# romanoshiliarhopoulos/Backgammon-Engine

Measured on AMD Instinct MI355X. Metric: self-play env steps/sec @65k concurrent games, higher is better.
Workload: dtype f32; 1 GPU; config3: 65 536 concurrent games per MI355X, greedy 198->128->1 value net (tdgammonNEW100k weights), auto-reset, Philox dice; games_per_gpu=65536, burnin_steps=160, parallelism=shard1, games_finished=2250605

## Files before the change

backgammon-engine_amd/csrc/bg_eval.h:

```cpp
#pragma once
#include "bg_board.h"
#include "bg_td_plan.h"

namespace bg {

constexpr int N_IN = 198, N_HID = 128;
constexpr int N_PARAMS = N_HID * N_IN + N_HID + N_HID + 1;
constexpr int K_STEPS = N_IN / 2;
constexpr int EVAL_LDS_BYTES = K_STEPS * 64 * 16;
constexpr int EVAL_THREADS = 768;

typedef float floatx16 __attribute__((ext_vector_type(16)));

__device__ __forceinline__ float fast_sigmoid(float x)
{
    return __builtin_amdgcn_rcpf(1.0f + __builtin_amdgcn_exp2f(-1.44269504088896340736f * x));
}

__device__ __forceinline__ void best_atomic_max(unsigned long long *__restrict__ best, uint32_t game, float v, uint32_t key_turn,
                                                bool valid, int width)
{
    const int lane = threadIdx.x & 63;
    uint32_t bits = __float_as_uint(v);
    bits = (key_turn >> 31) ? ~bits : bits;
// ... 415 lines not shown
            const uint32_t sd = mover ^ (uint32_t)pass;
            const uint32_t b0 = sd ? p[4] : p[0], b1 = sd ? p[5] : p[1], b2 = sd ? p[6] : p[2], b3 = sd ? p[7] : p[3];
            const uint32_t c0 = sd ? q[4] : q[0], c1 = sd ? q[5] : q[1], c2 = sd ? q[6] : q[2], c3 = sd ? q[7] : q[3];
            const uint32_t diff = (b0 ^ c0) | (b1 ^ c1) | (b2 ^ c2) | (b3 ^ c3);
            if (pass == 1 && __ballot(diff != 0u) == 0ull) break;
            const uint32_t ge_new[3] = {b0 | b1 | b2 | b3, b1 | b2 | b3, (b0 & b1) | b2 | b3};
            const uint32_t ge_old[3] = {c0 | c1 | c2 | c3, c1 | c2 | c3, (c0 & c1) | c2 | c3};
            const uint32_t side4 = 4u * sd;
#pragma unroll
            for (int k = 0; k < 3; ++k) {
                uint32_t x = (ge_new[k] ^ ge_old[k]) & PTS;
                while (x) {
                    const int pos = __ffs(x) - 1; x &= x - 1;
                    BG_PUSH(delta_row_board(pos - 1, 0) + side4 + (uint32_t)k, 0, ((ge_new[k] >> pos) & 1u) ? 1 : -1);
                }
            }
            uint32_t x4 = diff & PTS & ((b2 | b3) | (c2 | c3));
            const Side sn{{b0, b1, b2, b3}}, so{{c0, c1, c2, c3}};
            while (x4) {
                const int pos = __ffs(x4) - 1; x4 &= x4 - 1;
                const int n1 = count_at(sn, pos), n0 = count_at(so, pos);
                const int d = (n1 > 3 ? n1 - 3 : 0) - (n0 > 3 ? n0 - 3 : 0);
                if (d) BG_PUSH(delta_row_board(pos - 1, 0) + side4 + 3u, 1, d);
            }
            if (diff & 1u) {
                const int d = count_at(sn, 0) - count_at(so, 0);
                BG_PUSH(sd ? (uint32_t)delta_row(197) : (uint32_t)delta_row(194), 1, sd ? 2 * d : d);
            }
            if (diff & (1u << 25)) {
                const int d = count_at(sn, 25) - count_at(so, 25);
                BG_PUSH(sd ? (uint32_t)delta_row(195) : (uint32_t)delta_row(196), 1, sd ? d : 2 * d);
            }
        }
#else
#pragma unroll
        for (int sd = 0; sd < 2; ++sd) {
            const uint32_t b0 = p[4 * sd], b1 = p[4 * sd + 1], b2 = p[4 * sd + 2], b3 = p[4 * sd + 3];
            const uint32_t c0 = q[4 * sd], c1 = q[4 * sd + 1], c2 = q[4 * sd + 2], c3 = q[4 * sd + 3];
            const uint32_t diff = (b0 ^ c0) | (b1 ^ c1) | (b2 ^ c2) | (b3 ^ c3);
            const uint32_t ge_new[3] = {b0 | b1 | b2 | b3, b1 | b2 | b3, (b0 & b1) | b2 | b3};
            const uint32_t ge_old[3] = {c0 | c1 | c2 | c3, c1 | c2 | c3, (c0 & c1) | c2 | c3};
#pragma unroll
            for (int k = 0; k < 3; ++k) {
                uint32_t x = (ge_new[k] ^ ge_old[k]) & PTS;
                while (x) {
                    const int pos = __ffs(x) - 1; x &= x - 1;
                    BG_PUSH(delta_row_board(pos - 1, 4 * sd + k), 0, ((ge_new[k] >> pos) & 1u) ? 1 : -1);
                }
            }
            uint32_t x4 = diff & PTS & ((b2 | b3) | (c2 | c3));
            const Side sn{{b0, b1, b2, b3}}, so{{c0, c1, c2, c3}};
            while (x4) {
                const int pos = __ffs(x4) - 1; x4 &= x4 - 1;
                const int n1 = count_at(sn, pos), n0 = count_at(so, pos);
                const int d = (n1 > 3 ? n1 - 3 : 0) - (n0 > 3 ? n0 - 3 : 0);
                if (d) BG_PUSH(delta_row_board(pos - 1, 4 * sd + 3), 1, d);
            }
            if (diff & 1u) {
                const int d = count_at(sn, 0) - count_at(so, 0);
                BG_PUSH(delta_row(sd == 0 ? 194 : 197), sd == 0 ? 1 : 2, d);
            }
            if (diff & (1u << 25)) {
                const int d = count_at(sn, 25) - count_at(so, 25);
                BG_PUSH(delta_row(sd == 0 ? 196 : 195), sd == 0 ? 2 : 1, d);
            }
        }
#endif
        }
#undef BG_PUSH
        if (cnt > DELTA_MAX) { cnt = DELTA_MAX; list_overflow = true; }
        n_delta += cnt;
        uint32_t maxcnt = 0;
#pragma unroll
        for (int b = 4; b >= 0; --b) {
            const uint32_t t = maxcnt | (1u << b);
            if (__ballot(cnt >= t) != 0ull) maxcnt = t;
        }
#if defined(BG_ABL) && (BG_ABL & 2)
        maxcnt = maxcnt > 100 ? 1 : 0;
#endif
        __builtin_amdgcn_wave_barrier();

        f32x2_t sum2 = {0.0f, 0.0f};
        const f32x4_t *w2v = reinterpret_cast<const f32x4_t *>(sW2);
        const uint32_t sW_lds = (uint32_t)(uintptr_t)(__attribute__((address_space(3))) float4 *)sW;
#pragma unroll 1
        for (int c = 0; c < 2; ++c) {
            f32x2_t a[16], a2[16];
#if defined(BG_ABL) && (BG_ABL & 8)
#pragma unroll
            for (int j = 0; j < 16; ++j) { a[j] = (f32x2_t){0.25f * (float)j, 0.5f}; a2[j] = (f32x2_t){0.125f, -0.25f * (float)j}; }
            (void)ah;
#else
#pragma unroll
            for (int j = 0; j < 8; ++j) { const f32x4_t t = ah[16 * c + j]; a[2 * j] = t.lo; a[2 * j + 1] = t.hi; }
#pragma unroll
            for (int j = 0; j < 8; ++j) { const f32x4_t t = ah[16 * c + 8 + j]; a2[2 * j] = t.lo; a2[2 * j + 1] = t.hi; }
#endif
            if (c == 1) { nr0 = root_rows[2 * (long long)nxi.x]; nr1 = root_rows[2 * (long long)nxi.x + 1]; }
            uint32_t ent = lst[0];
            for (uint32_t e = 0; e < maxcnt; ++e) {
                const uint32_t nent = lst[(e + 1 < DELTA_MAX ? e + 1 : e) * 64];
                f32x2_t d2;
                uint32_t addr;
                delta_entry(ent, sW_lds + 256u * (uint32_t)c, d2, addr);
                delta_apply_32<0>(a, d2, addr);
                delta_apply_32<128>(a2, d2, addr);
                ent = nent;
            }
#if defined(BG_ABL) && (BG_ABL & 4)
#define BG_SIGP(A, W, S) __builtin_elementwise_fma(W, A, S)
#else
#define BG_SIGP(A, W, S) delta_sigmoid_pair(A, W, S)
#endif
#pragma unroll
            for (int j = 0; j < 8; ++j) {
                const f32x4_t w = w2v[16 * c + j];
                sum2 = BG_SIGP(a[2 * j], w.lo, sum2);
                sum2 = BG_SIGP(a[2 * j + 1], w.hi, sum2);
            }
#pragma unroll
            for (int j = 0; j < 8; ++j) {
                const f32x4_t w = w2v[16 * c + 8 + j];
                sum2 = BG_SIGP(a2[2 * j], w.lo, sum2);
                sum2 = BG_SIGP(a2[2 * j + 1], w.hi, sum2);
            }
#undef BG_SIGP
        }
        const float sum = sum2.x + sum2.y;
        __builtin_amdgcn_wave_barrier();
        {
            const float v = fast_sigmoid(sum + b2);
            if (valid) values[row] = v;
            best_atomic_max(best, __shfl(inf.x, inv, 64), __shfl(v, inv, 64), __shfl(inf.y, inv, 64), __shfl((int)valid, inv, 64) != 0, 64);
        }
        tile = next_tile;
    }
    __shared__ unsigned int s_nd;
    if (threadIdx.x == 0) s_nd = 0;
    __syncthreads();
    {
        uint32_t t = n_delta;
#pragma unroll
        for (int m = 1; m < 64; m <<= 1) t += __shfl_xor(t, m, 64);
        if (lane == 0 && t) atomicAdd(&s_nd, t);
    }
    __syncthreads();
    if (delta_counter && threadIdx.x == 0 && s_nd) atomicAdd(delta_counter, (unsigned long long)s_nd);
    if (err_word && __ballot(list_overflow) != 0ull && lane == 0) atomicOr(err_word, err_bit);
#ifdef BG_EVAL_WGCLOCK
    if (n_rows_ptr && threadIdx.x == 0) {
        values[n_rows_imm - 1 - (long long)blockIdx.x] = (float)(wall_clock64() - wg_t0) * 0.01f;
        values[n_rows_imm - 1 - (long long)gridDim.x - (long long)blockIdx.x] = (float)s_ticket;
    }
#endif
}

constexpr int K16_STEPS = 13;
constexpr int EVAL16_W_BYTES = K16_STEPS * 4 * 64 * 16;
constexpr int EVAL16_LUT_BYTES = 16 * 8;
constexpr int EVAL16_LDS_TOTAL = EVAL16_W_BYTES + EVAL16_LUT_BYTES + (EVAL_THREADS / 64) * EVAL_RED_FLOATS * 4;
typedef __bf16 bf16x8 __attribute__((ext_vector_type(8)));

__host__ __device__ inline uint16_t f32_to_bf16_rne(float f)
{
    union { float f; uint32_t u; } c{f};
    return (uint16_t)((c.u + 0x7FFFu + ((c.u >> 16) & 1u)) >> 16);
}

inline void relayout_w1_bf16(const float *w1, uint16_t *wl)
{
    for (int s = 0; s < K16_STEPS; ++s)
        for (int c = 0; c < 4; ++c)
            for (int l = 0; l < 64; ++l)
                for (int j = 0; j < 8; ++j) {
                    const int f = 16 * s + 8 * (l >> 5) + j;
                    wl[((s * 4 + c) * 64 + l) * 8 + j] = f < N_IN ? f32_to_bf16_rne(w1[(32 * c + (l & 31)) * N_IN + f]) : 0;
                }
}
inline void make_count_lut(uint32_t *lut )
{
    for (int n = 0; n < 16; ++n) {
        const uint16_t e0 = n >= 1 ? 0x3F80 : 0, e1 = n >= 2 ? 0x3F80 : 0, e2 = n >= 3 ? 0x3F80 : 0;
        const uint16_t e3 = n >= 4 ? f32_to_bf16_rne(0.5f * (float)(n - 3)) : 0;
        lut[2 * n] = (uint32_t)e0 | ((uint32_t)e1 << 16);
        lut[2 * n + 1] = (uint32_t)e2 | ((uint32_t)e3 << 16);
    }
}

__global__ __launch_bounds__(EVAL_THREADS) void eval_rows_bf16_kernel(
    const uint4 *__restrict__ rows, const unsigned long long *__restrict__ n_rows_ptr, long long n_rows_imm,
    unsigned long long *__restrict__ rows_eval_counter, const uint4 *__restrict__ wl16, const uint2 *__restrict__ lut,
    const float *__restrict__ b1, const float *__restrict__ w2, const float *__restrict__ b2p, float *__restrict__ values,
    const uint2 *__restrict__ info, unsigned long long *__restrict__ best)
{
    extern __shared__ uint4 sW16[];
    uint2 *sLut = reinterpret_cast<uint2 *>(sW16 + K16_STEPS * 4 * 64);
    float *sRed = reinterpret_cast<float *>(sLut + 16) + (threadIdx.x >> 6) * EVAL_RED_FLOATS;
    for (int i = threadIdx.x; i < K16_STEPS * 4 * 64; i += EVAL_THREADS) sW16[i] = wl16[i];
    if (threadIdx.x < 16) sLut[threadIdx.x] = lut[threadIdx.x];
    __syncthreads();

    long long n_rows = n_rows_imm;
    if (n_rows_ptr) { const long long c = (long long)*n_rows_ptr; n_rows = c < n_rows_imm ? c : n_rows_imm; }
    if (rows_eval_counter && blockIdx.x == 0 && threadIdx.x == 0) atomicAdd(rows_eval_counter, (unsigned long long)n_rows);
    const long long n_tiles = (n_rows + 31) >> 5;
    const int lane = threadIdx.x & 63;
    const int r = lane & 31, h = lane >> 5;
    const long long wave = (long long)blockIdx.x * (EVAL_THREADS / 64) + (threadIdx.x >> 6);
    const long long n_waves = (long long)gridDim.x * (EVAL_THREADS / 64);
    constexpr float NL2E = -1.44269504088896340736f;
    float b1s[4], w2v[4];
#pragma unroll
    for (int c = 0; c < 4; ++c) { b1s[c] = NL2E * b1[32 * c + r]; w2v[c] = w2[32 * c + r]; }
    const float b2 = *b2p;

    uint4 nx0 = make_uint4(0, 0, 0, 0), nx1 = make_uint4(0, 0, 0, 0);
    if (wave < n_tiles && wave * 32 + r < n_rows) { nx0 = rows[2 * (wave * 32 + r)]; nx1 = rows[2 * (wave * 32 + r) + 1]; }

    for (long long tile = wave; tile < n_tiles; tile += n_waves) {
        const uint32_t p[8] = {nx0.x, nx0.y, nx0.z, nx0.w, nx1.x, nx1.y, nx1.z, nx1.w};
        {
            const long long nrow = (tile + n_waves) * 32 + r;
            nx0 = make_uint4(0, 0, 0, 0); nx1 = make_uint4(0, 0, 0, 0);
            if (nrow < n_rows) { nx0 = rows[2 * nrow]; nx1 = rows[2 * nrow + 1]; }
        }
        const Side sa{{p[0], p[1], p[2], p[3]}}, sb{{p[4], p[5], p[6], p[7]}};
        floatx16 acc0 = {0}, acc1 = {0}, acc2 = {0}, acc3 = {0};
        const uint4 *wp = sW16 + lane;
#pragma unroll 4
        for (int s = 0; s < 12; ++s) {
            const int pos = 2 * s + h + 1;
            const uint2 l0 = sLut[count_at(sa, pos)], l1 = sLut[count_at(sb, pos)];
            union { uint4 u; bf16x8 v; } a, w0, w1, w2r, w3;
            a.u = make_uint4(l0.x, l0.y, l1.x, l1.y);
            w0.u = wp[(s * 4 + 0) * 64]; w1.u = wp[(s * 4 + 1) * 64]; w2r.u = wp[(s * 4 + 2) * 64]; w3.u = wp[(s * 4 + 3) * 64];
            acc0 = __builtin_amdgcn_mfma_f32_32x32x16_bf16(a.v, w0.v, acc0, 0, 0, 0);
            acc1 = __builtin_amdgcn_mfma_f32_32x32x16_bf16(a.v, w1.v, acc1, 0, 0, 0);
            acc2 = __builtin_amdgcn_mfma_f32_32x32x16_bf16(a.v, w2r.v, acc2, 0, 0, 0);
            acc3 = __builtin_amdgcn_mfma_f32_32x32x16_bf16(a.v, w3.v, acc3, 0, 0, 0);
        }
        {
            const int turn = (p[0] & TURN_BIT) ? 1 : 0;
            const uint32_t t0 = turn == 0 ? 0x3F80u : 0u, t1 = turn == 0 ? 0u : 0x3F80u;
            const uint32_t bar1 = f32_to_bf16_rne(0.5f * (float)count_at(sa, 0)), bar2 = f32_to_bf16_rne(0.5f * (float)count_at(sb, 25));
            const uint32_t off1 = f32_to_bf16_rne((float)count_at(sa, 25) / 15.0f), off2 = f32_to_bf16_rne((float)count_at(sb, 0) / 15.0f);
            union { uint4 u; bf16x8 v; } a, w0, w1, w2r, w3;
            a.u = h ? make_uint4(0, 0, 0, 0) : make_uint4(t0 | (t1 << 16), bar1 | (bar2 << 16), off1 | (off2 << 16), 0u);
            w0.u = wp[(12 * 4 + 0) * 64]; w1.u = wp[(12 * 4 + 1) * 64]; w2r.u = wp[(12 * 4 + 2) * 64]; w3.u = wp[(12 * 4 + 3) * 64];
            acc0 = __builtin_amdgcn_mfma_f32_32x32x16_bf16(a.v, w0.v, acc0, 0, 0, 0);
            acc1 = __builtin_amdgcn_mfma_f32_32x32x16_bf16(a.v, w1.v, acc1, 0, 0, 0);
            acc2 = __builtin_amdgcn_mfma_f32_32x32x16_bf16(a.v, w2r.v, acc2, 0, 0, 0);
            acc3 = __builtin_amdgcn_mfma_f32_32x32x16_bf16(a.v, w3.v, acc3, 0, 0, 0);
        }
        float part[16];
#pragma unroll
        for (int j = 0; j < 16; ++j) {
            const float s0 = __builtin_amdgcn_rcpf(1.0f + __builtin_amdgcn_exp2f(__builtin_fmaf(acc0[j], NL2E, b1s[0])));
            const float s1 = __builtin_amdgcn_rcpf(1.0f + __builtin_amdgcn_exp2f(__builtin_fmaf(acc1[j], NL2E, b1s[1])));
            const float s2 = __builtin_amdgcn_rcpf(1.0f + __builtin_amdgcn_exp2f(__builtin_fmaf(acc2[j], NL2E, b1s[2])));
            const float s3 = __builtin_amdgcn_rcpf(1.0f + __builtin_amdgcn_exp2f(__builtin_fmaf(acc3[j], NL2E, b1s[3])));
            part[j] = w2v[0] * s0 + w2v[1] * s1 + w2v[2] * s2 + w2v[3] * s3;
        }
#pragma unroll
        for (int q = 0; q < 4; ++q)
#pragma unroll
            for (int j = 0; j < 4; ++j) sRed[r * EVAL_RED_STRIDE + 8 * q + 4 * h + j] = part[4 * q + j];
        __builtin_amdgcn_wave_barrier();
        float sum = 0.0f;
#pragma unroll
        for (int c = 0; c < 16; ++c) sum += sRed[(16 * h + c) * EVAL_RED_STRIDE + r];
        sum += __shfl_xor(sum, 32, 64);
        __builtin_amdgcn_wave_barrier();
        {
            const long long orow = tile * 32 + r;
            const bool vrow = h == 0 && orow < n_rows;
            const float v = fast_sigmoid(sum + b2);
            if (vrow) values[orow] = v;
            if (info) {
                const uint2 inf = vrow ? info[orow] : make_uint2(0u, 0u);
                best_atomic_max(best, inf.x, v, inf.y, vrow, 32);
            }
        }
    }
}

#ifndef BG_ROOT3_PHASE_STEPS
#define BG_ROOT3_PHASE_STEPS 7
#endif
constexpr int ROOT3_PHASE_STEPS = BG_ROOT3_PHASE_STEPS;
constexpr int ROOT3_PHASES = (K16_STEPS + ROOT3_PHASE_STEPS - 1) / ROOT3_PHASE_STEPS;
constexpr int ROOT3_PART_U4 = K16_STEPS * 4 * 64;
constexpr int ROOT3_LDS_TOTAL = 3 * ROOT3_PHASE_STEPS * 4 * 64 * 16 + EVAL16_LUT_BYTES;

inline void relayout_w1_bf16x3(const float *w1, uint16_t *wl)
{
    static const int tail_map[8] = {192, 193, 194, 195, 196, 197, -1, -1};
    for (int s = 0; s < K16_STEPS; ++s)
        for (int c = 0; c < 4; ++c)
            for (int l = 0; l < 64; ++l)
                for (int j = 0; j < 8; ++j) {
                    int f = 16 * s + 8 * (l >> 5) + j;
                    if (s == 12) f = (l >> 5) == 0 ? tail_map[j] : -1;
                    float w = f >= 0 && f < N_IN ? w1[(32 * c + (l & 31)) * N_IN + f] : 0.0f;
                    if (f >= 196) w = w / 15.0f;
                    const size_t o = (((size_t)s * 4 + c) * 64 + l) * 8 + j;
// ... 386 lines not shown
```

backgammon-engine_amd/csrc/bg_root_resident.h:

```cpp
#pragma once
#include "bg_eval.h"

namespace bg {

constexpr int D16_XBUF_U4 = K16_STEPS * 64;

#ifndef BG_ROOT_F16X2
#define BG_ROOT_F16X2 1
#endif
#if BG_ROOT_F16X2
constexpr int ROOT_PLANES = 2;
typedef f16x8 root_vec8;
#define BG_ROOT_MFMA(A, B, C) __builtin_amdgcn_mfma_f32_32x32x16_f16(A, B, C, 0, 0, 0)
__device__ __forceinline__ uint32_t root_half_bits(float x) { return (uint32_t)f16_bits((_Float16)x); }
constexpr uint32_t ROOT_ONE = 0x3C00u;
#else
constexpr int ROOT_PLANES = 3;
typedef bf16x8 root_vec8;
#define BG_ROOT_MFMA(A, B, C) __builtin_amdgcn_mfma_f32_32x32x16_bf16(A, B, C, 0, 0, 0)
__device__ __forceinline__ uint32_t root_half_bits(float x) { return (uint32_t)f32_to_bf16_rne(x); }
constexpr uint32_t ROOT_ONE = 0x3F80u;
#endif
constexpr bool ROOT_F16X2 = BG_ROOT_F16X2 != 0;

__host__ __device__ inline bool w1_fits_f16_split(float w, _Float16 &hi, _Float16 &lo)
{
    const float aw = w < 0.0f ? -w : w;
    hi = (_Float16)w;
    lo = (_Float16)(w - (float)hi);
    const float res = w - ((float)hi + (float)lo);
    return aw < 65504.0f
           && (res < 0.0f ? -res : res) <= aw * 4.76837158e-7f + 5.96046448e-8f;
}

inline int relayout_w1_f16x2_root(const float *w1, uint16_t *wl)
{
    static const int tail_map[8] = {192, 193, 194, 195, 196, 197, -1, -1};
    int rc = 0;
    for (int s = 0; s < K16_STEPS; ++s)
        for (int c = 0; c < 4; ++c)
            for (int l = 0; l < 64; ++l)
                for (int j = 0; j < 8; ++j) {
                    int f = 16 * s + 8 * (l >> 5) + j;
                    if (s == 12) f = (l >> 5) == 0 ? tail_map[j] : -1;
                    float w = f >= 0 && f < N_IN ? w1[(32 * c + (l & 31)) * N_IN + f] : 0.0f;
                    if (f >= 196) w = w / 15.0f;
                    _Float16 hi, lo;
                    if (!w1_fits_f16_split(w, hi, lo)) rc = -1;
                    const size_t o = (((size_t)s * 4 + c) * 64 + l) * 8 + j;
                    wl[o] = f16_bits(hi);
                    wl[(size_t)ROOT3_PART_U4 * 8 + o] = f16_bits(lo);
                }
    return rc;
}

constexpr int ROOTR_THREADS = 256;
constexpr int ROOTR_LDS_BYTES = 2 * D16_XBUF_U4 * 16 + EVAL16_LUT_BYTES + 3 * 1024;

__global__ __launch_bounds__(ROOTR_THREADS, 2) void root_hidden_resident_kernel(
    const uint4 *__restrict__ rows, long long n_rows, const uint4 *__restrict__ wl3, const uint2 *__restrict__ lut,
    const float *__restrict__ b1, float *__restrict__ hidden)
{
    extern __shared__ uint4 sRR[];
    uint4 *sX = sRR;
    uint2 *sLut = reinterpret_cast<uint2 *>(sX + 2 * D16_XBUF_U4);
    uint4 *sRows = reinterpret_cast<uint4 *>(sLut + 16);
    if (threadIdx.x < 16) sLut[threadIdx.x] = lut[threadIdx.x];
    const int lane = threadIdx.x & 63, c = __builtin_amdgcn_readfirstlane((int)(threadIdx.x >> 6));
    const int r = lane & 31, h = lane >> 5;
    const long long n_tiles = (n_rows + 31) >> 5;
    union WF { uint4 u; root_vec8 v; };
    WF wf[ROOT_PLANES][K16_STEPS];
#pragma unroll
    for (int p = 0; p < ROOT_PLANES; ++p)
#pragma unroll
        for (int s = 0; s < K16_STEPS; ++s) wf[p][s].u = wl3[(size_t)p * ROOT3_PART_U4 + ((size_t)s * 4 + c) * 64 + lane];
    constexpr float NL2E = -1.44269504088896340736f;
    const float bb = b1[32 * c + r];
    __syncthreads();

    auto fetch = [&](long long tile, int slot) {
        if (c == 0 && tile * 32 + (lane >> 1) < n_rows)
            __builtin_amdgcn_global_load_lds((const __attribute__((address_space(1))) void *)(rows + tile * 64 + lane),
                                             (__attribute__((address_space(3))) void *)(sRows + slot * 64), 16, 0, 0);
    };
    auto stage = [&](long long tile, int buf, int slot) {
        uint32_t p[8] = {0, 0, 0, 0, 0, 0, 0, 0};
        const bool row_ok = tile < n_tiles && tile * 32 + r < n_rows;
        if (row_ok) {
            const uint4 u0 = sRows[slot * 64 + 2 * r], u1 = sRows[slot * 64 + 2 * r + 1];
            p[0] = u0.x; p[1] = u0.y; p[2] = u0.z; p[3] = u0.w; p[4] = u1.x; p[5] = u1.y; p[6] = u1.z; p[7] = u1.w;
        }
        const Side sa{{p[0], p[1], p[2], p[3]}}, sb{{p[4], p[5], p[6], p[7]}};
        uint4 *dst = sX + buf * D16_XBUF_U4 + lane;
#pragma unroll
        for (int q = 0; q < 3; ++q) {
            const int pos = 2 * (c + 4 * q) + h + 1;
            const uint2 l0 = sLut[count_at(sa, pos)], l1 = sLut[count_at(sb, pos)];
            dst[(c + 4 * q) * 64] = make_uint4(l0.x, l0.y, l1.x, l1.y);
        }
        if (c == 0) {
            const int turn = (p[0] & TURN_BIT) ? 1 : 0;
            const uint32_t t0 = (turn == 0 && row_ok) ? ROOT_ONE : 0u, t1 = (turn == 0 || !row_ok) ? 0u : ROOT_ONE;
            const uint32_t bar1 = root_half_bits(0.5f * (float)count_at(sa, 0)), bar2 = root_half_bits(0.5f * (float)count_at(sb, 25));
            const uint32_t off1 = root_half_bits((float)count_at(sa, 25)), off2 = root_half_bits((float)count_at(sb, 0));
            dst[12 * 64] = h ? make_uint4(0, 0, 0, 0) : make_uint4(t0 | (t1 << 16), bar1 | (bar2 << 16), off1 | (off2 << 16), 0u);
        }
    };

    long long tile = blockIdx.x;
    fetch(tile, 0);
    fetch(tile + gridDim.x, 1);
    asm volatile("s_waitcnt vmcnt(0)" ::: "memory");
    __syncthreads();
    stage(tile, 0, 0);
    __syncthreads();
    int it = 0, slot = 0;
    for (; tile < n_tiles; tile += gridDim.x, ++it) {
        const int buf = it & 1;
        const int slot1 = slot == 2 ? 0 : slot + 1, slot2 = slot1 == 2 ? 0 : slot1 + 1;
        fetch(tile + 2 * (long long)gridDim.x, slot2);
        stage(tile + gridDim.x, buf ^ 1, slot1);
        floatx16 acc = {0};
        const uint4 *xp = sX + buf * D16_XBUF_U4 + lane;
#pragma unroll
        for (int s = 0; s < K16_STEPS; ++s) {
            WF x;
            x.u = xp[s * 64];
#pragma unroll
            for (int p = 0; p < ROOT_PLANES; ++p) acc = BG_ROOT_MFMA(x.v, wf[p][s].v, acc);
        }
#pragma unroll
        for (int j = 0; j < 16; ++j) {
            const long long orow = tile * 32 + (j & 3) + 8 * (j >> 2) + 4 * h;
            if (orow < n_rows) hidden[orow * N_HID + 32 * c + r] = NL2E * (acc[j] + bb);
        }
        asm volatile("s_waitcnt vmcnt(0)" ::: "memory");
        __syncthreads();
        slot = slot1;
    }
}


constexpr int BROOT_THREADS = 256;
#ifndef BG_BROOT_GPW
#define BG_BROOT_GPW 128
#endif
constexpr int BROOT_GPW = BG_BROOT_GPW;
constexpr int BROOT_TILES = BROOT_GPW / 32;
constexpr int BROOT_LDS_BYTES = BROOT_TILES * D16_XBUF_U4 * 16 + EVAL16_LUT_BYTES + BROOT_GPW * 32;

struct BRootWeights { uint4 w[ROOT_PLANES][K16_STEPS]; };

__device__ __forceinline__ void broot_load_weights(const uint4 *__restrict__ wl3, BRootWeights &wf)
{
    const int lane = threadIdx.x & 63, c = __builtin_amdgcn_readfirstlane((int)(threadIdx.x >> 6));
#pragma unroll
    for (int p = 0; p < ROOT_PLANES; ++p)
#pragma unroll
#if defined(BG_ABL_STEP) && (BG_ABL_STEP & 8)
        for (int s = 0; s < K16_STEPS; ++s) wf.w[p][s] = make_uint4(lane + s, p, c, 0u);
#else
        for (int s = 0; s < K16_STEPS; ++s) wf.w[p][s] = wl3[(size_t)p * ROOT3_PART_U4 + ((size_t)s * 4 + c) * 64 + lane];
#endif
}

__device__ __forceinline__ int boundary_root_stage(uint4 row0, uint4 row1, long long g0, long long n_games, const uint2 *__restrict__ lut)
{
    extern __shared__ uint4 sBR[];
    uint4 *sX = sBR;
    uint2 *sLut = reinterpret_cast<uint2 *>(sX + BROOT_TILES * D16_XBUF_U4);
    uint4 *sRows = reinterpret_cast<uint4 *>(sLut + 16);
    if (threadIdx.x < 16) sLut[threadIdx.x] = lut[threadIdx.x];
    if (threadIdx.x < BROOT_GPW) {
        sRows[2 * threadIdx.x] = row0;
        sRows[2 * threadIdx.x + 1] = row1;
    }
    const int lane = threadIdx.x & 63, c = __builtin_amdgcn_readfirstlane((int)(threadIdx.x >> 6));
    const int r = lane & 31, h = lane >> 5;
    long long left = n_games - g0;
    const int n_tiles = left <= 0 ? 0 : (int)((left < BROOT_GPW ? left : BROOT_GPW) + 31) >> 5;
    __syncthreads();
    for (int tile = 0; tile < n_tiles; ++tile) {
        uint32_t p[8] = {0, 0, 0, 0, 0, 0, 0, 0};
        const bool row_ok = g0 + tile * 32 + r < n_games;
        if (row_ok) {
            const uint4 u0 = sRows[2 * (tile * 32 + r)], u1 = sRows[2 * (tile * 32 + r) + 1];
            p[0] = u0.x; p[1] = u0.y; p[2] = u0.z; p[3] = u0.w; p[4] = u1.x; p[5] = u1.y; p[6] = u1.z; p[7] = u1.w;
        }
        const Side sa{{p[0], p[1], p[2], p[3]}}, sb{{p[4], p[5], p[6], p[7]}};
        uint4 *dst = sX + tile * D16_XBUF_U4 + lane;
#pragma unroll
        for (int q = 0; q < 3; ++q) {
            const int pos = 2 * (c + 4 * q) + h + 1;
            const uint2 l0 = sLut[count_at(sa, pos)], l1 = sLut[count_at(sb, pos)];
            dst[(c + 4 * q) * 64] = make_uint4(l0.x, l0.y, l1.x, l1.y);
        }
        if (c == 0) {
            const int turn = (p[0] & TURN_BIT) ? 1 : 0;
            const uint32_t t0 = (turn == 0 && row_ok) ? ROOT_ONE : 0u, t1 = (turn == 0 || !row_ok) ? 0u : ROOT_ONE;
            const uint32_t bar1 = root_half_bits(0.5f * (float)count_at(sa, 0)), bar2 = root_half_bits(0.5f * (float)count_at(sb, 25));
            const uint32_t off1 = root_half_bits((float)count_at(sa, 25)), off2 = root_half_bits((float)count_at(sb, 0));
            dst[12 * 64] = h ? make_uint4(0, 0, 0, 0) : make_uint4(t0 | (t1 << 16), bar1 | (bar2 << 16), off1 | (off2 << 16), 0u);
        }
    }
    return n_tiles;
}

__device__ __forceinline__ void boundary_root_compute(const BRootWeights &wf, int n_tiles, long long g0, long long n_games,
                                                      const float *__restrict__ b1, float *__restrict__ hidden)
{
    extern __shared__ uint4 sBR[];
    uint4 *sX = sBR;
    const int lane = threadIdx.x & 63, c = __builtin_amdgcn_readfirstlane((int)(threadIdx.x >> 6));
    const int r = lane & 31, h = lane >> 5;
    constexpr float NL2E = -1.44269504088896340736f;
    const float bb = b1[32 * c + r];
    __syncthreads();
    union WF { uint4 u; root_vec8 v; };
#if defined(BG_ABL_STEP) && (BG_ABL_STEP & 2)
    if (n_tiles > 100)
#endif
    for (int tile = 0; tile < n_tiles; tile += 2) {
        floatx16 acc0 = {0}, acc1 = {0};
        const uint4 *xp0 = sX + tile * D16_XBUF_U4 + lane;
        const uint4 *xp1 = sX + (tile + 1 < n_tiles ? tile + 1 : tile) * D16_XBUF_U4 + lane;
#pragma unroll
        for (int s = 0; s < K16_STEPS; ++s) {
            WF x0, x1;
            x0.u = xp0[s * 64];
            x1.u = xp1[s * 64];
#pragma unroll
            for (int p = 0; p < ROOT_PLANES; ++p) {
                WF wv;
                wv.u = wf.w[p][s];
                acc0 = BG_ROOT_MFMA(x0.v, wv.v, acc0);
                acc1 = BG_ROOT_MFMA(x1.v, wv.v, acc1);
            }
        }
#pragma unroll
        for (int j = 0; j < 16; ++j) {
            const long long orow = g0 + tile * 32 + (j & 3) + 8 * (j >> 2) + 4 * h;
#if defined(BG_ABL_STEP) && (BG_ABL_STEP & 4)
            if (acc0[j] == 1.2345f || acc1[j] == 1.2345f) hidden[orow * N_HID + 32 * c + r] = 0.0f;
#else
            if (orow < n_games) hidden[orow * N_HID + 32 * c + r] = NL2E * (acc0[j] + bb);
            if (tile + 1 < n_tiles && orow + 32 < n_games) hidden[(orow + 32) * N_HID + 32 * c + r] = NL2E * (acc1[j] + bb);
#endif
        }
    }
}

}
```

backgammon-engine_amd/csrc/bg_staged_kernels.h:

```cpp
#pragma once

struct NodeState {
    Side own, opp;
    int pl, dA, dB, len;
    bool dbl;
};

__device__ __forceinline__ void node_build(const Node &nd, const uint32_t (&p)[8], uint32_t meta, NodeState &s,
                                           Side *before_last_own = nullptr, Side *before_last_opp = nullptr)
{
    s.pl = meta & 1;
    const int d1 = (meta >> 4) & 7, d2 = (meta >> 8) & 7;
    const int pass = key_pass(nd.key);
    s.dA = pass ? d2 : d1;
    s.dB = pass ? d1 : d2;
    s.dbl = d1 == d2;
    s.len = key_len(nd.key);
    split_sides(p, s.pl, s.own, s.opp);
#pragma unroll
    for (int k = 0; k < 3; ++k)
        if (k < s.len) {
            if (before_last_own && k == s.len - 1) { *before_last_own = s.own; *before_last_opp = s.opp; }
            apply_move(s.own, s.opp, s.pl, key_origin(nd.key, k), (k & 1) ? s.dB : s.dA);
        }
// ... 349 lines not shown
                chain->pown = a; chain->popp = b;
                bool hit = (pk & 0x01000000u) != 0;
                if (o != 31) {
                    const int dest = pl ? o - die : o + die;
                    if (dest >= 1 && dest <= 24) hit = hit || (((b.b[0] & ~(b.b[1] | b.b[2] | b.b[3])) >> dest) & 1u);
                    apply_move(a, b, pl, o, die);
                    key = key_child(key, o);
                }
                chain->hit = hit;
                chain->own = a; chain->opp = b; chain->game = game; chain->key = key; chain->pl = pl; chain->die = die;
                chain->valid = true;
                continue;
            }
            if (o != 31) {
                apply_move(a, b, pl, o, die);
                key = key_child(key, o);
            }
            const unsigned long long d = two ? (q >= totA ? (unsigned long long)(ar0 + 1) * sv.b_base + baseB2 + (q - totA)
                                                           : (unsigned long long)ar0 * sv.b_base + baseA + q)
                                             : baseA + (q - q0);
            if (MODE == MODE_LEAF) {
                const Side &s1 = pl ? b : a, &s2 = pl ? a : b;
                sv.u_rows[2 * d] = make_uint4(s1.b[0] | (pl ? TURN_BIT : 0u), s1.b[1], s1.b[2], s1.b[3]);
                sv.u_rows[2 * d + 1] = make_uint4(s2.b[0], s2.b[1], s2.b[2], s2.b[3]);
                sv.u_info[d] = make_uint2(game, key | (pl ? 0x80000000u : 0u));
            } else if (MODE == MODE_PLY2) sv.d2[d] = Node{game, key};
            else lp.list[d] = Node{game, key};
        }
    }
    block_barrier<PH_LDS && (MODE == MODE_LEAF || CHAIN)>();
    BG_PSTAMP(3);
#undef BG_PSTAMP
    *out_base = baseA;
    *out_total = ok ? listed : 0u;
    if (out_all) *out_all = ok ? total : 0u;
}

template <int MODE, int NT, bool STUCK_ROWS = false, bool CHAIN = false>
__device__ __forceinline__ void expand_phase(const EnvView &e, const StagedView &sv, const NodeIn &x, int np,
                                             unsigned long long *out_base, uint32_t *out_total, const LeafParents &lp,
                                             ExpandLds<NT> &L, uint32_t *out_stuck = nullptr, ChainNode *chain = nullptr,
                                             uint32_t *out_all = nullptr, bool kind_dbl = false)
{
    (void)np;
    NodeState s;
    s.own = s.opp = Side{{0, 0, 0, 0}};
    s.pl = 0; s.dA = s.dB = 1; s.len = 0; s.dbl = false;
    Side prev_own{{0, 0, 0, 0}}, prev_opp{{0, 0, 0, 0}};
    bool prefix_hit = false;
    if (x.valid) {
        node_build(x.nd, x.pl, x.meta, s, &prev_own, &prev_opp);
        Side rown, ropp;
        split_sides(x.pl, s.pl, rown, ropp);
        const int bar = s.pl ? 0 : 25;
        prefix_hit = ((((s.opp.b[0] ^ ropp.b[0]) | (s.opp.b[1] ^ ropp.b[1]) | (s.opp.b[2] ^ ropp.b[2]) | (s.opp.b[3] ^ ropp.b[3])) >> bar) & 1u) != 0;
    }
    expand_phase_core<MODE, NT, STUCK_ROWS, CHAIN>(e, sv, x.valid, x.nd, s, prev_own, prev_opp, x.pl, prefix_hit, out_base, out_total, lp, L,
                                                   out_stuck, chain, out_all, kind_dbl);
}

template <int MODE, int NT>
__device__ __forceinline__ void expand_phase_chained(const EnvView &e, const StagedView &sv, const ChainNode &n,
                                                     unsigned long long *out_base, uint32_t *out_total, const LeafParents &lp,
                                                     ExpandLds<NT> &L, ChainNode *chain, uint32_t *out_all)
{
    NodeState s;
    s.own = n.own; s.opp = n.opp; s.pl = n.pl; s.dA = s.dB = n.die; s.dbl = true; s.len = key_len(n.key);
    const uint32_t no_root[8] = {0, 0, 0, 0, 0, 0, 0, 0};
    expand_phase_core<MODE, NT, false, MODE != MODE_LEAF>(e, sv, n.valid, Node{n.game, n.key}, s, n.pown, n.popp, no_root, n.valid && n.hit, out_base,
                                                          out_total, lp, L, nullptr, chain, out_all, true);
}

__device__ __forceinline__ unsigned long long nodes_per_block(unsigned long long n_in, int nt)
{
    unsigned long long npb = (n_in + gridDim.x - 1) / gridDim.x;
    npb = (npb + 63) & ~63ull;
    return npb < 64 ? 64 : (npb > (unsigned long long)nt ? (unsigned long long)nt : npb);
}

#ifdef BGAMD_EXPERIMENTAL
template <int MODE>
__global__ __launch_bounds__(expand_threads(MODE)) void expand_kernel(EnvView e, StagedView sv)
{
    constexpr int NT = expand_threads(MODE);
    __shared__ ExpandLds<NT> L;
    const Node *in = MODE == MODE_PLY2 ? sv.d1 : (MODE == MODE_PLY3 ? sv.d2 : sv.f);
    const unsigned long long cap_in = (unsigned long long)(MODE == MODE_PLY2 ? sv.cap_d1 : (MODE == MODE_PLY3 ? sv.cap_d2 : sv.cap_f));
    unsigned long long n_in = sv.tops[MODE == MODE_PLY2 ? T_D1 : (MODE == MODE_PLY3 ? T_D2 : T_F)];
    if (n_in > cap_in) n_in = cap_in;
    unsigned long long staged_total = 0;
    if (MODE == MODE_LEAF && blockIdx.x == 0 && threadIdx.x == 0) {
        atomicAdd(&e.counters[C_FNODES], n_in);
        atomicAdd(&e.counters[C_DNODES], sv.tops[T_D1] + sv.tops[T_D2]);
    }
    const unsigned long long NPB = nodes_per_block(n_in, NT);
    auto idx_of = [&](unsigned long long blk) -> long long {
        const unsigned long long node = blk * NPB + threadIdx.x;
        return (threadIdx.x < NPB && node < n_in) ? (long long)node : -1ll;
    };
    NodeIn cur, nxt;
    node_fetch(e, in, blockIdx.x * NPB < n_in ? idx_of(blockIdx.x) : -1ll, cur);
    for (unsigned long long blk = blockIdx.x; blk * NPB < n_in; blk += gridDim.x) {
        const unsigned long long nb = blk + gridDim.x;
        node_fetch(e, in, nb * NPB < n_in ? idx_of(nb) : -1ll, nxt);
        unsigned long long base;
        uint32_t total;
        expand_phase<MODE, NT>(e, sv, cur, (int)NPB, &base, &total, leaf_parents_shared(sv), L);
        staged_total += total;
        cur = nxt;
    }
    if (MODE == MODE_LEAF && threadIdx.x == 0 && staged_total) atomicAdd(&e.counters[C_CAND_RAW], staged_total);
}

__global__ __launch_bounds__(expand_threads(MODE_PLY2)) void doubles_kernel(EnvView e, StagedView sv)
{
    constexpr int NT = expand_threads(MODE_PLY2);
    __shared__ ExpandLds<NT> L;
    unsigned long long n_in = sv.tops[T_D1];
    if (n_in > (unsigned long long)sv.cap_d1) n_in = (unsigned long long)sv.cap_d1;
    const unsigned long long NPB = nodes_per_block(n_in, NT / 4);
    for (unsigned long long blk = blockIdx.x; blk * NPB < n_in; blk += gridDim.x) {
        const unsigned long long first = blk * NPB;
        const unsigned long long cnt = n_in - first < NPB ? n_in - first : NPB;
        unsigned long long base2;
        uint32_t total2;
        NodeIn x2;
        node_fetch(e, sv.d1, threadIdx.x < cnt ? (long long)(first + threadIdx.x) : -1ll, x2);
        expand_phase<MODE_PLY2, NT>(e, sv, x2, (int)NPB, &base2, &total2, leaf_parents_shared(sv), L);
        for (uint32_t c = 0; c < total2; c += NT) {
            const unsigned long long n3 = total2 - c < (uint32_t)NT ? total2 - c : (uint32_t)NT;
            unsigned long long base3;
            uint32_t total3;
            NodeIn x3;
            node_fetch(e, sv.d2, threadIdx.x < n3 ? (long long)(base2 + c + threadIdx.x) : -1ll, x3);
            expand_phase<MODE_PLY3, NT>(e, sv, x3, NT, &base3, &total3, leaf_parents_shared(sv), L);
        }
    }
}
#endif

#ifndef BG_XALL_NT
#define BG_XALL_NT 512
#endif
constexpr int XALL_NT = BG_XALL_NT;
__global__ __launch_bounds__(XALL_NT, 4) void expand_all_kernel(EnvView e, StagedView sv, unsigned n_dbl, unsigned dbl_npb, unsigned parts,
                                                                  unsigned long long *__restrict__ zero_words, int n_zero_words)
{
    constexpr int NT = XALL_NT;
    if (zero_words && blockIdx.x == gridDim.x - 1 && (int)threadIdx.x < n_zero_words) zero_words[threadIdx.x] = 0ull;
    __shared__ ExpandLds<NT> L;
#ifdef BG_EVAL_WGCLOCK
    const unsigned long long xall_t0 = wall_clock64();
    if (threadIdx.x == 0) for (int k = 0; k < 8; ++k) e.values[e.cap - 1 - 4096 - (long long)blockIdx.x * 8 - k] = 0.0f;
#endif
    uint32_t acc_staged = 0, acc_fnodes = 0, acc_dnodes = 0;
    auto add_staged = [&](unsigned long long v) { acc_staged += (uint32_t)v; };
    auto add_fnodes = [&](unsigned long long v) { acc_fnodes += (uint32_t)v; };
    auto add_dnodes = [&](unsigned long long v) { acc_dnodes += (uint32_t)v; };
    const bool do_dbl = blockIdx.x < n_dbl && (parts & 1u), do_leaf = blockIdx.x >= n_dbl && (parts & 2u);
    if (do_dbl) {
        const LeafParents lp{sv.f2, &sv.tops[T_F2], (unsigned long long)sv.cap_f2};
        const int shd = sv.shards > 1 ? (int)(blockIdx.x % (unsigned)sv.shards) : 0;
        const unsigned long long capD = (unsigned long long)(sv.cap_d1 / sv.shards);
        const Node *d1_list = sv.d1 + (unsigned long long)shd * capD;
        unsigned long long n_in = sv.tops[d1_counter(shd)];
        if (n_in > capD) n_in = capD;
        const unsigned long long d_first = (unsigned long long)blockIdx.x / (unsigned)sv.shards, d_stride = (unsigned long long)n_dbl / (unsigned)sv.shards;
        if (d_first == 0) add_dnodes(n_in);
        unsigned long long NPB = (n_in + d_stride - 1) / d_stride;
        NPB = NPB < 1 ? 1 : (NPB > (unsigned long long)dbl_npb ? (unsigned long long)dbl_npb : NPB);
        auto leaf_range = [&](unsigned long long base, uint32_t n) {
            for (uint32_t c4 = 0; c4 < n; c4 += NT) {
                const unsigned long long n4 = n - c4 < (uint32_t)NT ? n - c4 : (uint32_t)NT;
                unsigned long long base4;
                uint32_t total4;
                NodeIn x4;
                node_fetch(e, sv.f2, threadIdx.x < n4 ? (long long)(base + c4 + threadIdx.x) : -1ll, x4);
                expand_phase<MODE_LEAF, NT>(e, sv, x4, NT, &base4, &total4, lp, L, nullptr, nullptr, nullptr, true);
                add_staged(total4);
            }
        };
        for (unsigned long long blk = d_first; blk * NPB < n_in; blk += d_stride) {
            const unsigned long long first = blk * NPB;
            const unsigned long long cnt = n_in - first < NPB ? n_in - first : NPB;
            unsigned long long over2_base, over3_base, base4;
            uint32_t over2, over3, all2, all3, total4, stuck2;
            NodeIn x2;
            ChainNode n3, n4;
            node_fetch(e, d1_list, threadIdx.x < cnt ? (long long)(first + threadIdx.x) : -1ll, x2);
            expand_phase<MODE_PLY2, NT, true, true>(e, sv, x2, (int)NPB, &over2_base, &over2, lp, L, &stuck2, &n3, &all2);
            add_dnodes(all2);
            add_fnodes(stuck2);
            add_staged(stuck2);
            expand_phase_chained<MODE_PLY3, NT>(e, sv, n3, &over3_base, &over3, lp, L, &n4, &all3);
            add_fnodes(all3);
            expand_phase_chained<MODE_LEAF, NT>(e, sv, n4, &base4, &total4, lp, L, nullptr, nullptr);
            add_staged(total4);
            if (over2 | over3) __syncthreads();
            leaf_range(over3_base, over3);
            for (uint32_t c = 0; c < over2; c += NT) {
                const unsigned long long n3c = over2 - c < (uint32_t)NT ? over2 - c : (uint32_t)NT;
                unsigned long long base3;
                uint32_t total3;
                NodeIn x3;
                node_fetch(e, sv.d2, threadIdx.x < n3c ? (long long)(over2_base + c + threadIdx.x) : -1ll, x3);
                expand_phase<MODE_PLY3, NT>(e, sv, x3, NT, &base3, &total3, lp, L);
                add_fnodes(total3);
                leaf_range(base3, total3);
            }
        }
    }
    if (do_leaf) {
        const unsigned int lw = blockIdx.x - n_dbl;
        const int shf = sv.shards > 1 ? (int)(lw % (unsigned)sv.shards) : 0;
        const unsigned long long capF = (unsigned long long)(sv.cap_f / sv.shards);
        const Node *f_list = sv.f + (unsigned long long)shf * capF;
        unsigned long long n_in = sv.tops[f_counter(shf)];
        if (n_in > capF) n_in = capF;
        const unsigned long long l_first = lw / (unsigned)sv.shards, l_stride = (unsigned long long)(gridDim.x - n_dbl) / (unsigned)sv.shards;
        if (l_first == 0) add_fnodes(n_in);
        const unsigned long long share = (n_in + l_stride - 1) / l_stride;
        const unsigned long long lo = l_first * share < n_in ? l_first * share : n_in;
        const unsigned long long hi = lo + share < n_in ? lo + share : n_in;
        const unsigned long long chunks = (hi - lo + NT - 1) / NT;
        const unsigned long long per = chunks ? (hi - lo + chunks - 1) / chunks : 0;
        auto idx_of = [&](unsigned long long c) -> long long {
            const unsigned long long node = lo + c * per + threadIdx.x;
            return (c < chunks && threadIdx.x < per && node < hi) ? (long long)node : -1ll;
        };
        NodeIn cur, nxt;
        node_fetch(e, f_list, idx_of(0), cur);
        for (unsigned long long c = 0; c < chunks; ++c) {
            node_fetch(e, f_list, idx_of(c + 1), nxt);
            unsigned long long base;
            uint32_t total;
            expand_phase<MODE_LEAF, NT>(e, sv, cur, (int)per, &base, &total, leaf_parents_shared(sv), L);
            add_staged(total);
            cur = nxt;
        }
    }
    if (threadIdx.x == 0) {
        const unsigned long long staged_total = acc_staged, fnodes = acc_fnodes, dnodes = acc_dnodes;
        if (staged_total) atomicAdd(&e.counters[C_CAND_RAW], staged_total);
        if (fnodes) atomicAdd(&e.counters[C_FNODES], fnodes);
        if (dnodes) atomicAdd(&e.counters[C_DNODES], dnodes);
#ifdef BG_EVAL_WGCLOCK
        e.values[e.cap - 1 - 1024 - (long long)blockIdx.x] = (float)(wall_clock64() - xall_t0) * 0.01f;
        e.values[e.cap - 1 - 2048 - (long long)blockIdx.x] = (float)staged_total;
#endif
    }
}

struct IndexVisitor {
    uint32_t n = 0, idx = 0xFFFFFFFFu, t_orig, t_len, t_dA, t_dB;
    __device__ __forceinline__ bool leaf(const Side &, const Side &, uint32_t origins, int len, int dA, int dB)
    {
        if (origins == t_orig && (uint32_t)len == t_len && (uint32_t)dA == t_dA && (uint32_t)dB == t_dB) idx = n;
        ++n;
        return false;
    }
};

struct ExploreView {
    const Node *tasks; const uint32_t *task_count, *task_off, *task_n;
};
__device__ __forceinline__ bool explore_pick(const EnvView &e, const ExploreView &xv, long long g, uint32_t u, Side &own,
                                             Side &opp, uint32_t &key, uint32_t &k, uint32_t &C);

__device__ __forceinline__ void apply_body(const EnvView &e, const StagedView &sv, const ExploreView &xv, int flags, float epsilon,
                                           long long g, LaneCtx *fwd = nullptr)
{
    LaneCtx c;
    lane_begin(e, g, flags & ~BGAMD_ROLL, c);
    const unsigned long long pack = (g < e.n && c.live) ? sv.best[g] : 0ull;
    const bool has = pack != 0ull;
    int32_t chosen = -1;
    uint32_t cseq = 0, ccount = has ? 1u : 0u;
    float cval = 0.0f;
    if (has) {
        Side own, opp;
        split_sides(c.p, c.turn, own, opp);
        const bool explore = epsilon > 0.0f && (float)(c.x.w >> 8) * (1.0f / 16777216.0f) < epsilon;
        uint32_t key = ~(uint32_t)pack & 0x7FFFFFFFu;
        const uint32_t vb = (uint32_t)(pack >> 32);
        cval = __uint_as_float(c.turn ? ~vb : vb);
        uint32_t xk = 0, xC = 0;
        const bool explored = explore && explore_pick(e, xv, g, c.x.z, own, opp, key, xk, xC);
        {
            const int len = key_len(key), pass = key_pass(key);
            const int dA = pass ? c.d2 : c.d1, dB = pass ? c.d1 : c.d2;
            uint32_t origins = 0;
#pragma unroll
            for (int k = 0; k < 4; ++k)
                if (k < len) origins |= (uint32_t)key_origin(key, k) << (5 * k);
            if (explored) { chosen = (int32_t)xk; ccount = xC; cval = 0.0f; }
            else if (flags & BGAMD_WANT_INDEX) {
                IndexVisitor iv;
                iv.t_orig = origins; iv.t_len = (uint32_t)len; iv.t_dA = (uint32_t)dA; iv.t_dB = (uint32_t)dB;
                walk_sequences(own, opp, c.turn, c.d1, c.d2, iv);
                chosen = (int32_t)iv.idx; ccount = iv.n;
            } else chosen = 0;
            if (!explored) {
#pragma unroll
                for (int k = 0; k < 4; ++k)
                    if (k < len) apply_move(own, opp, c.turn, key_origin(key, k), (k & 1) ? dB : dA);
            }
            cseq = seq_pack(origins, len, dA, dB) | (c.turn ? (1u << 29) : 0u);
        }
        join_sides(own, opp, c.turn, c.p);
    }
    if (c.live) { e.chosen[g] = chosen; e.chosen_seq[g] = cseq; e.chosen_val[g] = cval; e.cand_cnt[g] = ccount; }
    uint32_t after[3] = {c.meta, c.ply, c.epi};
    finish_turn(e, g, c.p, c.turn, c.d1, c.d2, c.ply, c.epi, flags, c.live, after);
    if (fwd) {
#pragma unroll
        for (int k = 0; k < 8; ++k) fwd->p[k] = c.p[k];
        fwd->meta = after[0]; fwd->ply = after[1]; fwd->epi = after[2];
    }
}

__global__ __launch_bounds__(LANE_NT) void apply_kernel(EnvView e, StagedView sv, ExploreView xv, int flags, float epsilon)
{
    apply_body(e, sv, xv, flags, epsilon, (long long)blockIdx.x * LANE_NT + threadIdx.x);
}

template <bool ROOT>
__global__ __launch_bounds__(LANE_NT, 2) void boundary_kernel(EnvView e, StagedView sv, StagedView sv_next, ExploreView xv, int flags,
                                                           float epsilon, const uint4 *__restrict__ wl3, const uint2 *__restrict__ lut,
                                                           const float *__restrict__ b1)
{
    static_assert(!ROOT || LANE_NT == BROOT_THREADS, "the in-launch root pass is written for 256-thread workgroups");
    constexpr int GPW = ROOT ? BROOT_GPW : LANE_NT;
    const long long g = (int)threadIdx.x < GPW ? (long long)blockIdx.x * GPW + threadIdx.x : e.n;
    LaneCtx next;
    apply_body(e, sv, xv, flags, epsilon, g, &next);
    __syncthreads();
    uint4 row[2];
    BRootWeights wf;
    if (ROOT) broot_load_weights(wl3, wf);
    RootsPending P;
    roots_issue(e, sv_next, flags, g, &next, ROOT ? row : nullptr, P);
#if defined(BG_ALLOC_DEFERRED) && !BG_ALLOC_DEFERRED
    roots_collect(e, sv_next, P);
#endif
    int n_tiles = 0;
    if (ROOT) n_tiles = boundary_root_stage(row[0], row[1], (long long)blockIdx.x * GPW, e.n, lut);
#if !defined(BG_ALLOC_DEFERRED) || BG_ALLOC_DEFERRED
    roots_collect(e, sv_next, P);
#endif
    if (ROOT) boundary_root_compute(wf, n_tiles, (long long)blockIdx.x * GPW, e.n, b1, sv_next.root_hidden);
}
```

Before: 540.6 million env steps/s.

## Pace root MFMA chains with staggered tiles and streamed hidden stores

```diff
diff --git a/backgammon-engine_amd/csrc/bg_eval.h b/backgammon-engine_amd/csrc/bg_eval.h
--- a/backgammon-engine_amd/csrc/bg_eval.h
+++ b/backgammon-engine_amd/csrc/bg_eval.h
@@ -591,6 +591,8 @@
     if (n_rows_ptr && threadIdx.x == 0) {
         values[n_rows_imm - 1 - (long long)blockIdx.x] = (float)(wall_clock64() - wg_t0) * 0.01f;
         values[n_rows_imm - 1 - (long long)gridDim.x - (long long)blockIdx.x] = (float)s_ticket;
+        values[n_rows_imm - 1 - 10240 - (long long)blockIdx.x] = __uint_as_float((uint32_t)wg_t0);
+        values[n_rows_imm - 1 - 11264 - (long long)blockIdx.x] = __uint_as_float((uint32_t)wall_clock64());
     }
 #endif
 }
diff --git a/backgammon-engine_amd/csrc/bg_root_resident.h b/backgammon-engine_amd/csrc/bg_root_resident.h
--- a/backgammon-engine_amd/csrc/bg_root_resident.h
+++ b/backgammon-engine_amd/csrc/bg_root_resident.h
@@ -1,5 +1,6 @@
 #pragma once
 #include "bg_eval.h"
+#include "bg_stream_store.h"
 
 namespace bg {
 
@@ -207,6 +208,76 @@
     return n_tiles;
 }
 
+template <bool FULL>
+__device__ __forceinline__ void broot_paced_chains(const BRootWeights &wf, int n_tiles, int lim, const uint4 *sXl, float bb, float *hp)
+{
+    constexpr int ROUNDS = (BROOT_TILES + 1) / 2, LAG = K16_STEPS / 2, NSLOT = ROUNDS * K16_STEPS + LAG, PER = (16 + LAG - 1) / LAG;
+    static_assert(2 * LAG <= K16_STEPS && PER * LAG >= 16, "a tile's stores leave before the other chain's tile ends");
+    constexpr float NL2E = -1.44269504088896340736f;
+    union WF { uint4 u; root_vec8 v; };
+    floatx16 accA = {0}, accB = {0};
+    float pend[16];
+    auto put = [&](int tile, int j, float v) {
+        const int orow = tile * 32 + (j & 3) + 8 * (j >> 2);
+#if defined(BG_ABL_STEP) && (BG_ABL_STEP & 4)
+        if (v == 1.2345f) hp[(long long)orow * N_HID] = 0.0f;
+#else
+        if (FULL || (tile < n_tiles && orow < lim)) stream_store(hp + (long long)orow * N_HID, v);
+#endif
+    };
+    auto drain = [&](int tile, int j0) {
+#pragma unroll
+        for (int j = PER; j < 16; ++j)
+            if (j >= j0 && j < j0 + PER) put(tile, j, pend[j]);
+    };
+    auto finish = [&](int tile, const floatx16 &acc) {
+#pragma unroll
+        for (int j = 0; j < 16; ++j) {
+            const float v = NL2E * (acc[j] + bb);
+            if (j < PER) put(tile, j, v);
+            else pend[j] = v;
+        }
+    };
+#pragma unroll
+    for (int t = 0; t < NSLOT; ++t) {
+        if (t >= K16_STEPS) {
+            const int d = (t - K16_STEPS) % K16_STEPS, k2 = 2 * ((t - K16_STEPS) / K16_STEPS);
+            if (d < LAG) drain(k2, PER * (d + 1));
+            else if (d < 2 * LAG) drain(k2 + 1, PER * (d - LAG + 1));
+        }
+        const int tA = 2 * (t / K16_STEPS), sA = t % K16_STEPS;
+        const int tB = 2 * ((t - LAG) / K16_STEPS) + 1, sB = (t - LAG) % K16_STEPS;
+        const bool onA = t < ROUNDS * K16_STEPS, onB = t >= LAG && tB < BROOT_TILES;
+        if (onA && (FULL || tA < n_tiles)) {
+            if (sA == 0) accA = floatx16{0};
+            WF x;
+            x.u = sXl[tA * D16_XBUF_U4 + sA * 64];
+#pragma unroll
+            for (int p = 0; p < ROOT_PLANES; ++p) {
+                WF wv;
+                wv.u = wf.w[p][sA];
+                accA = BG_ROOT_MFMA(x.v, wv.v, accA);
+            }
+        }
+        if (onB && (FULL || tB < n_tiles)) {
+            if (sB == 0) accB = floatx16{0};
+            WF x;
+            x.u = sXl[tB * D16_XBUF_U4 + sB * 64];
+#pragma unroll
+            for (int p = 0; p < ROOT_PLANES; ++p) {
+                WF wv;
+                wv.u = wf.w[p][sB];
+                accB = BG_ROOT_MFMA(x.v, wv.v, accB);
+            }
+        }
+        if (onA && sA == K16_STEPS - 1 && (FULL || tA < n_tiles)) finish(tA, accA);
+        if (onB && sB == K16_STEPS - 1 && (FULL || tB < n_tiles)) finish(tB, accB);
+    }
+    if (2 * ROUNDS <= BROOT_TILES)
+#pragma unroll
+        for (int j0 = PER; j0 < 16; j0 += PER) drain(2 * ROUNDS - 1, j0);
+}
+
 __device__ __forceinline__ void boundary_root_compute(const BRootWeights &wf, int n_tiles, long long g0, long long n_games,
                                                       const float *__restrict__ b1, float *__restrict__ hidden)
 {
@@ -214,41 +285,18 @@
     uint4 *sX = sBR;
     const int lane = threadIdx.x & 63, c = __builtin_amdgcn_readfirstlane((int)(threadIdx.x >> 6));
     const int r = lane & 31, h = lane >> 5;
-    constexpr float NL2E = -1.44269504088896340736f;
     const float bb = b1[32 * c + r];
     __syncthreads();
-    union WF { uint4 u; root_vec8 v; };
 #if defined(BG_ABL_STEP) && (BG_ABL_STEP & 2)
     if (n_tiles > 100)
 #endif
-    for (int tile = 0; tile < n_tiles; tile += 2) {
-        floatx16 acc0 = {0}, acc1 = {0};
-        const uint4 *xp0 = sX + tile * D16_XBUF_U4 + lane;
-        const uint4 *xp1 = sX + (tile + 1 < n_tiles ? tile + 1 : tile) * D16_XBUF_U4 + lane;
-#pragma unroll
-        for (int s = 0; s < K16_STEPS; ++s) {
-            WF x0, x1;
-            x0.u = xp0[s * 64];
-            x1.u = xp1[s * 64];
-#pragma unroll
-            for (int p = 0; p < ROOT_PLANES; ++p) {
-                WF wv;
-                wv.u = wf.w[p][s];
-                acc0 = BG_ROOT_MFMA(x0.v, wv.v, acc0);
-                acc1 = BG_ROOT_MFMA(x1.v, wv.v, acc1);
-            }
-        }
-#pragma unroll
-        for (int j = 0; j < 16; ++j) {
-            const long long orow = g0 + tile * 32 + (j & 3) + 8 * (j >> 2) + 4 * h;
-#if defined(BG_ABL_STEP) && (BG_ABL_STEP & 4)
-            if (acc0[j] == 1.2345f || acc1[j] == 1.2345f) hidden[orow * N_HID + 32 * c + r] = 0.0f;
-#else
-            if (orow < n_games) hidden[orow * N_HID + 32 * c + r] = NL2E * (acc0[j] + bb);
-            if (tile + 1 < n_tiles && orow + 32 < n_games) hidden[(orow + 32) * N_HID + 32 * c + r] = NL2E * (acc1[j] + bb);
-#endif
-        }
-    }
-}
-
-}
+    {
+        const long long left = n_games - g0 - 4 * h;
+        const int lim = left > BROOT_GPW ? BROOT_GPW : (int)left;
+        float *hp = hidden + (g0 + 4 * h) * N_HID + 32 * c + r;
+        if (n_tiles == BROOT_TILES && g0 + BROOT_GPW <= n_games) broot_paced_chains<true>(wf, n_tiles, lim, sX + lane, bb, hp);
+        else broot_paced_chains<false>(wf, n_tiles, lim, sX + lane, bb, hp);
+    }
+}
+
+}
diff --git a/backgammon-engine_amd/csrc/bg_staged_kernels.h b/backgammon-engine_amd/csrc/bg_staged_kernels.h
--- a/backgammon-engine_amd/csrc/bg_staged_kernels.h
+++ b/backgammon-engine_amd/csrc/bg_staged_kernels.h
@@ -525,6 +525,7 @@
 #ifdef BG_EVAL_WGCLOCK
     const unsigned long long xall_t0 = wall_clock64();
     if (threadIdx.x == 0) for (int k = 0; k < 8; ++k) e.values[e.cap - 1 - 4096 - (long long)blockIdx.x * 8 - k] = 0.0f;
+    if (threadIdx.x == 0) e.values[e.cap - 1 - 8192 - (long long)blockIdx.x] = __uint_as_float((uint32_t)xall_t0);
 #endif
     uint32_t acc_staged = 0, acc_fnodes = 0, acc_dnodes = 0;
     auto add_staged = [&](unsigned long long v) { acc_staged += (uint32_t)v; };
@@ -620,6 +621,7 @@
 #ifdef BG_EVAL_WGCLOCK
         e.values[e.cap - 1 - 1024 - (long long)blockIdx.x] = (float)(wall_clock64() - xall_t0) * 0.01f;
         e.values[e.cap - 1 - 2048 - (long long)blockIdx.x] = (float)staged_total;
+        e.values[e.cap - 1 - 9216 - (long long)blockIdx.x] = __uint_as_float((uint32_t)wall_clock64());
 #endif
     }
 }
@@ -703,6 +705,10 @@
                                                            const float *__restrict__ b1)
 {
     static_assert(!ROOT || LANE_NT == BROOT_THREADS, "the in-launch root pass is written for 256-thread workgroups");
+#ifdef BG_EVAL_WGCLOCK
+    if (threadIdx.x == 0)
+        e.values[e.cap - 1 - 12288 - (long long)blockIdx.x] = __uint_as_float((uint32_t)wall_clock64());
+#endif
     constexpr int GPW = ROOT ? BROOT_GPW : LANE_NT;
     const long long g = (int)threadIdx.x < GPW ? (long long)blockIdx.x * GPW + threadIdx.x : e.n;
     LaneCtx next;
@@ -722,4 +728,7 @@
     roots_collect(e, sv_next, P);
 #endif
     if (ROOT) boundary_root_compute(wf, n_tiles, (long long)blockIdx.x * GPW, e.n, b1, sv_next.root_hidden);
-}
+#ifdef BG_EVAL_WGCLOCK
+    if (threadIdx.x == 0) e.values[e.cap - 1 - 13312 - (long long)blockIdx.x] = __uint_as_float((uint32_t)wall_clock64());
+#endif
+}
diff --git a/backgammon-engine_amd/csrc/bg_stream_store.h b/backgammon-engine_amd/csrc/bg_stream_store.h
--- /dev/null
+++ b/backgammon-engine_amd/csrc/bg_stream_store.h
@@ -0,0 +1,19 @@
+#pragma once
+#include <hip/hip_runtime.h>
+
+#ifndef BG_STREAM_STORES
+#define BG_STREAM_STORES 1
+#endif
+
+namespace bg {
+
+__device__ __forceinline__ void stream_store(float *p, float v)
+{
+#if BG_STREAM_STORES
+    asm volatile("global_store_dword %0, %1, off sc1\n\ts_nop 1" : : "v"(p), "v"(v) : "memory");
+#else
+    *p = v;
+#endif
+}
+
+}
```

After: 551.8 million env steps/s, median of 6. 1.02x the previous value.
